# Zialus/CUDA-Recommender

Hardware: AMD Instinct MI355X
Metric: rating-nnz/sec per CCD++ outer iter at k=64 (higher is better)
Workload: dtype f32

## Files before the change

### cuda-recommender_amd/csrc/ccd_kernels.hip

```cpp
#include "ccd_kernels.hpp"

#include <algorithm>
#include <cstdlib>
#include <mutex>
#include <type_traits>

#include "flat_layout.hpp"

namespace mfx {
namespace {

constexpr int kBlock = 256;
constexpr uint32_t kPerSegLdsCap = 1024;

using u32x4 = __attribute__((ext_vector_type(4))) uint32_t;
using f32x4 = __attribute__((ext_vector_type(4))) float;
using u16x4 = __attribute__((ext_vector_type(4))) uint16_t;

template <int CTRL, int ROW_MASK = 0xF>
__device__ __forceinline__ float dpp_mov(float src) {
    return __builtin_bit_cast(float, __builtin_amdgcn_update_dpp(0, __builtin_bit_cast(int, src), CTRL, ROW_MASK, 0xF, true));
}
constexpr int kDppRowShr = 0x110, kDppWaveShr1 = 0x138, kDppBcast15 = 0x142, kDppBcast31 = 0x143;

__device__ __forceinline__ float wave_sum(float x) {
    const uint32_t lane = threadIdx.x & 63;
    x += dpp_mov<kDppRowShr + 1>(x);
    x += dpp_mov<kDppRowShr + 2>(x);
    x += dpp_mov<kDppRowShr + 4>(x);
    x += dpp_mov<kDppRowShr + 8>(x);
    const float r15 = dpp_mov<kDppBcast15, 0xA>(x);
    if (lane & 16) x += r15;
    const float r31 = dpp_mov<kDppBcast31, 0xC>(x);
    if (lane & 32) x += r31;
    return __builtin_bit_cast(float, __builtin_amdgcn_readlane(__builtin_bit_cast(int, x), 63));
}

__device__ __forceinline__ void seg_scan2(float& xg, float& xh, uint32_t lane, uint32_t dist) {
    const uint32_t in_row = lane & 15;
#define MFX_SCAN_STEP(D)                                                            \
    {                                                                               \
        const float yg = dpp_mov<kDppRowShr + D>(xg), yh = dpp_mov<kDppRowShr + D>(xh); \
        if (in_row >= D && dist >= D) { xg += yg; xh += yh; }                     \
    }
    MFX_SCAN_STEP(1) MFX_SCAN_STEP(2) MFX_SCAN_STEP(4) MFX_SCAN_STEP(8)
#undef MFX_SCAN_STEP
    {
        const float yg = dpp_mov<kDppBcast15, 0xA>(xg), yh = dpp_mov<kDppBcast15, 0xA>(xh);
        if ((lane & 16) && dist > in_row) { xg += yg; xh += yh; }
    }
    {
        const float yg = dpp_mov<kDppBcast31, 0xC>(xg), yh = dpp_mov<kDppBcast31, 0xC>(xh);
        if ((lane & 32) && dist > lane - 32) { xg += yg; xh += yh; }
    }
}

__device__ __forceinline__ float mul_rn(float a, float b) {
#pragma clang fp contract(off)
    return a * b;
}
__device__ __forceinline__ float add_rn(float a, float b) {
#pragma clang fp contract(off)
    return a + b;
}
__device__ __forceinline__ float sub_rn(float a, float b) {
#pragma clang fp contract(off)
    return a - b;
}

__global__ __launch_bounds__(kBlock) void k_sweep_wave(uint32_t nseg, const uint32_t* __restrict__ ptr,
                                                       const uint32_t* __restrict__ idx,
                                                       const float* __restrict__ val,
                                                       const float* __restrict__ vec,
                                                       float* __restrict__ g_out, float* __restrict__ h_out) {
    const uint32_t lane = threadIdx.x & 63;
    const uint32_t wave = (blockIdx.x * kBlock + threadIdx.x) >> 6;
    const uint32_t nwaves = (gridDim.x * kBlock) >> 6;
    for (uint32_t c = wave; c < nseg; c += nwaves) {
        const uint32_t lo = ptr[c], hi = ptr[c + 1];
        float g = 0.f, h = 0.f;
        for (uint32_t p = lo + lane; p < hi; p += 64) {
            const float x = vec[idx[p]];
            g += x * val[p];
            h += x * x;
        }
        g = wave_sum(g);
        h = wave_sum(h);
        if (lane == 0) {
            g_out[c] = g;
            h_out[c] = h;
        }
    }
}

__global__ __launch_bounds__(kBlock) void k_resid_wave(uint32_t nseg, const uint32_t* __restrict__ ptr,
                                                       const uint32_t* __restrict__ idx,
                                                       float* __restrict__ val,
                                                       const float* __restrict__ gathered,
                                                       const float* __restrict__ per_seg, int add) {
    const uint32_t lane = threadIdx.x & 63;
    const uint32_t wave = (blockIdx.x * kBlock + threadIdx.x) >> 6;
    const uint32_t nwaves = (gridDim.x * kBlock) >> 6;
    for (uint32_t c = wave; c < nseg; c += nwaves) {
        const uint32_t lo = ptr[c], hi = ptr[c + 1];
        const float b = per_seg[c];
        for (uint32_t p = lo + lane; p < hi; p += 64) {
            const float prod = mul_rn(gathered[idx[p]], b);
            val[p] = add ? add_rn(val[p], prod) : sub_rn(val[p], prod);
        }
    }
}

struct FlatArgs {
    const void* idx;
    float* val;
    const uint32_t* flags32;
    const uint32_t* hpre;
    const uint32_t* seg_of_rank;
    const uint32_t* wg_panel;
    uint32_t nspans;
    uint32_t tiles_per_span;
    uint32_t panel_rows;
    uint32_t gather_len;
    uint32_t nne;
    uint64_t nnz;
    const void* gather;
    const void* perseg;
    float2* part;
    float2* carry;
    int add;
    const uint32_t* wg_order;
    const uint32_t* wg_g0;
    const uint32_t* wg_g1;
    const uint32_t* expected;
    uint32_t* arrived;
    const uint32_t* orphans;
    uint32_t norphans, ngroups, panel_lanes;
    uint32_t nseg, npanels;
    const uint32_t* ptr_v;
    const uint32_t* rank_code;
    const uint32_t* seg_cnt;
    float lambda;
    float* out_vec;
    float2* pack2;
    const float* next_vec;
    float4* pack4;
    const float* gather_aux;
};

struct F3 { float x, y, z; };
template <typename S, typename G> __device__ __forceinline__ S to_slice(const G& g) { return g; }
template <> __device__ __forceinline__ F3 to_slice<F3, float4>(const float4& g) { return F3{g.x, g.y, g.z}; }
template <typename G, typename S> __device__ __forceinline__ G from_slice(const S& s) { return s; }
template <> __device__ __forceinline__ float4 from_slice<float4, F3>(const F3& s) { return make_float4(s.x, s.y, s.z, 0.f); }
template <int MODE> struct ModeTraits;
template <> struct ModeTraits<FM_SWEEP> { using G = float;  using S = float;  using P = float;  static constexpr bool kPerSeg = false, kWrite = false, kDot = true, kAux = false; };
template <> struct ModeTraits<FM_RESID> { using G = float;  using S = float;  using P = float;  static constexpr bool kPerSeg = true,  kWrite = true,  kDot = false, kAux = false; };
template <> struct ModeTraits<FM_FCSC>  { using G = float2; using S = float2; using P = float2; static constexpr bool kPerSeg = true,  kWrite = true,  kDot = true, kAux = false; };
template <> struct ModeTraits<FM_FCSR>  { using G = float4; using S = F3;     using P = float2; static constexpr bool kPerSeg = true,  kWrite = true,  kDot = true, kAux = false; };
template <> struct ModeTraits<FM_FCSC_RO> { using G = float2; using S = float2; using P = float2; static constexpr bool kPerSeg = true, kWrite = false, kDot = true, kAux = false; };
template <> struct ModeTraits<FM_FCSR_RO> { using G = float4; using S = F3;     using P = float2; static constexpr bool kPerSeg = true, kWrite = false, kDot = true, kAux = false; };
template <> struct ModeTraits<FM_FCSC2> { using G = float4; using S = float4; using P = float4; static constexpr bool kPerSeg = true,  kWrite = true,  kDot = true, kAux = false; };
template <> struct ModeTraits<FM_FCSR2> { using G = float4; using S = float4; using P = float4; static constexpr bool kPerSeg = true,  kWrite = true,  kDot = true, kAux = true; };

__device__ __forceinline__ float zero_of(float) { return 0.f; }
__device__ __forceinline__ float2 zero_of(float2) { return make_float2(0.f, 0.f); }
__device__ __forceinline__ float4 zero_of(float4) { return make_float4(0.f, 0.f, 0.f, 0.f); }

template <int MODE>
__device__ __forceinline__ void element_op(float v, const typename ModeTraits<MODE>::G& ga, float aux,
                                           const typename ModeTraits<MODE>::P& ps, int add,
                                           float& v_out, float& gc, float& hc) {
    if constexpr (MODE == FM_SWEEP) {
        v_out = v;
        gc = ga * v;
        hc = ga * ga;
    } else if constexpr (MODE == FM_RESID) {
        const float prod = mul_rn(ga, ps);
        v_out = add ? add_rn(v, prod) : sub_rn(v, prod);
        gc = 0.f;
        hc = 0.f;
    } else if constexpr (MODE == FM_FCSC || MODE == FM_FCSC_RO) {
        v_out = add_rn(sub_rn(v, mul_rn(ga.x, ps.x)), mul_rn(ga.y, ps.y));
        gc = ga.y * v_out;
        hc = ga.y * ga.y;
    } else if constexpr (MODE == FM_FCSR || MODE == FM_FCSR_RO) {
        v_out = add_rn(sub_rn(v, mul_rn(ga.x, ps.x)), mul_rn(ga.y, ps.y));
        gc = ga.z * v_out;
        hc = ga.z * ga.z;
    } else {
        const float r = add_rn(sub_rn(v, mul_rn(ga.x, ps.x)), mul_rn(ga.y, ps.y));
        v_out = add_rn(sub_rn(r, mul_rn(ga.z, ps.z)), mul_rn(ga.w, ps.w));
        const float d = MODE == FM_FCSC2 ? ga.w : aux;
        gc = d * v_out;
        hc = d * d;
    }
}

template <int BLOCK> __device__ void fused_finalize(const FlatArgs& a, uint32_t chunk, unsigned char* lds_raw);

using gu64 = __attribute__((address_space(1))) unsigned long long;
using gu32 = __attribute__((address_space(1))) uint32_t;
template <bool FUSE>
__device__ __forceinline__ void store_partial(float2* p, float g, float h) {
    if constexpr (FUSE) {
        const unsigned long long bits = (unsigned long long) __builtin_bit_cast(uint32_t, g) | ((unsigned long long) __builtin_bit_cast(uint32_t, h) << 32);
        __hip_atomic_store((gu64*) p, bits, __ATOMIC_RELAXED, __HIP_MEMORY_SCOPE_AGENT);
    } else {
        *p = make_float2(g, h);
    }
}
__device__ __forceinline__ float2 load_partial_sc1(const float2* p) {
    const unsigned long long bits = __hip_atomic_load((gu64*) p, __ATOMIC_RELAXED, __HIP_MEMORY_SCOPE_AGENT);
    return make_float2(__builtin_bit_cast(float, (uint32_t) bits), __builtin_bit_cast(float, (uint32_t) (bits >> 32)));
}

template <int MODE> constexpr int flat_min_waves(int block) { return MODE == FM_FCSC_RO || MODE == FM_FCSR_RO ? block / 128 : 1; }

#ifndef MFX_RO_PERSIST_FORM
#define MFX_RO_PERSIST_FORM 1
#endif
template <int MODE, bool LDS, int BLOCK, bool PSCHK, bool FUSE = false, bool PERSIST = false>
__global__ __launch_bounds__(BLOCK, flat_min_waves<MODE>(BLOCK)) void k_flat(FlatArgs a) {
    static_assert(!FUSE || ModeTraits<MODE>::kDot, "fused finalize: passes that produce sums");
    static_assert(!PERSIST || (LDS && !FUSE), "persistent form: LDS panels without the in-pass finalize");
    using TR = ModeTraits<MODE>;
    constexpr bool ROP = PERSIST && !TR::kWrite;
    constexpr bool PERSIST2 = PERSIST && TR::kWrite;
    uint32_t chunk = FUSE ? a.wg_order[blockIdx.x] : blockIdx.x;
    uint32_t chunk_end = chunk + 1;
    const uint32_t nchunks = a.nspans / (BLOCK / 64);
    if constexpr (PERSIST) {
        chunk = (uint32_t) ((uint64_t) blockIdx.x * nchunks / gridDim.x);
        chunk_end = (uint32_t) ((uint64_t) (blockIdx.x + 1) * nchunks / gridDim.x);
        if (chunk >= chunk_end) return;
    }
    using G = typename TR::G;
    using P = typename TR::P;
    extern __shared__ __attribute__((aligned(16))) unsigned char lds_raw[];
    using S = typename TR::S;
    S* __restrict__ slice = reinterpret_cast<S*>(lds_raw);
    constexpr size_t kSliceEntry = sizeof(S) + (TR::kAux ? sizeof(float) : 0);
    float* __restrict__ aux_slice = reinterpret_cast<float*>(lds_raw + ((size_t) a.panel_rows + 1) * sizeof(S));
    const uint32_t lane = threadIdx.x & 63;
    uint32_t span = __builtin_amdgcn_readfirstlane(chunk * (BLOCK / 64) + (threadIdx.x >> 6));
    const G* __restrict__ gather = static_cast<const G*>(a.gather);
    const P* __restrict__ perseg = static_cast<const P*>(a.perseg);
    const uint32_t span_words = a.tiles_per_span * (kTileElems / 32);
    uint64_t start = (uint64_t) span * a.tiles_per_span * kTileElems;
    using IdxVec = typename std::conditional<LDS, u16x4, u32x4>::type;
    using IdxElem = typename std::conditional<LDS, uint16_t, uint32_t>::type;
    const IdxVec* __restrict__ idx4 = reinterpret_cast<const IdxVec*>(static_cast<const IdxElem*>(a.idx) + start) + lane;
    f32x4* __restrict__ val4 = reinterpret_cast<f32x4*>(a.val + start) + lane;
    const uint32_t* __restrict__ flw = a.flags32 + (size_t) span * span_words + (lane >> 3);
    const uint32_t* __restrict__ hpw = a.hpre + (size_t) span * span_words + (lane >> 3);
    const uint32_t sh = (lane & 7) * 4;
    IdxVec id_n;
    f32x4 v_n;
    uint32_t fl_n, hp_n, hp_nn;
    const size_t span_step_q = (size_t) (BLOCK / 64) * a.tiles_per_span * 64, span_step_w = (size_t) (BLOCK / 64) * span_words;
    uint64_t sq = ROP ? (uint64_t) span * a.tiles_per_span * 64 : 0, sw = ROP ? (uint64_t) span * span_words : 0;
    struct LaneOff { uint32_t i, v, w; };
    auto lane_off = [](uint32_t lane) { LaneOff o{lane * (uint32_t) sizeof(IdxVec), lane * 16u, (lane >> 3) * 4u}; asm volatile("" : "+v"(o.i), "+v"(o.v), "+v"(o.w)); return o; };
    using gchar = __attribute__((address_space(1))) const char;
    auto ubase = [](const void* p) {
        const uint64_t u = reinterpret_cast<uint64_t>(p);
        return reinterpret_cast<gchar*>((uint64_t) (uint32_t) __builtin_amdgcn_readfirstlane((int) (u >> 32)) << 32 | (uint32_t) __builtin_amdgcn_readfirstlane((int) u));
    };
    using GIdxVec = __attribute__((address_space(1))) const IdxVec;
    using GF32x4 = __attribute__((address_space(1))) const f32x4;
    auto ld_idx = [&](uint64_t q, uint32_t lane_ib) { return __builtin_nontemporal_load(reinterpret_cast<GIdxVec*>(ubase(static_cast<const IdxVec*>(a.idx) + (sq + q)) + lane_ib)); };
    auto ld_val = [&](uint64_t q, uint32_t lane_vb) { return __builtin_nontemporal_load(reinterpret_cast<GF32x4*>(ubase(reinterpret_cast<const f32x4*>(a.val) + (sq + q)) + lane_vb)); };
    auto ld_fl = [&](uint64_t w, uint32_t lane_wb) { return *reinterpret_cast<const gu32*>(ubase(a.flags32 + (sw + w)) + lane_wb); };
    auto ld_hp = [&](uint64_t w, uint32_t lane_wb) { return *reinterpret_cast<const gu32*>(ubase(a.hpre + (sw + w)) + lane_wb); };
    auto stage_slice = [&](uint32_t panel) {
        const uint32_t gbase = panel * a.panel_rows;
        const uint32_t cnt = a.gather_len - gbase < a.panel_rows ? a.gather_len - gbase : a.panel_rows;
        for (uint32_t i = threadIdx.x; i < cnt; i += BLOCK) slice[i] = to_slice<S, G>(gather[gbase + i]);
        if (threadIdx.x == 0) slice[a.panel_rows] = S{};
        if constexpr (TR::kAux) {
            for (uint32_t i = threadIdx.x; i < cnt; i += BLOCK) aux_slice[i] = a.gather_aux[gbase + i];
            if (threadIdx.x == 0) aux_slice[a.panel_rows] = 0.f;
        }
    };
    uint32_t panel = 0, panel_next = 0;
    if constexpr (LDS) {
        id_n = __builtin_nontemporal_load(idx4);
        v_n = __builtin_nontemporal_load(val4);
        fl_n = flw[0]; hp_n = hpw[0]; hp_nn = hpw[8];
        panel = a.wg_panel[chunk];
        stage_slice(panel);
    }
    P* __restrict__ ps_lds = reinterpret_cast<P*>(lds_raw + (((size_t) a.panel_rows + 1) * kSliceEntry + 15) / 16 * 16);
    uint32_t win_base = 0;
    auto heads_before = [&](uint32_t c) { return a.hpre[(size_t) c * (BLOCK / 64) * span_words]; };
    uint32_t hb1 = 0, hb2 = 0;
    if constexpr (LDS && TR::kPerSeg) {
        const uint32_t rb0 = heads_before(chunk);
        win_base = rb0 > 0 ? rb0 - 1 : 0;
        const uint32_t win_end = heads_before(chunk + 1);
        if constexpr (PERSIST2) { hb1 = win_end; hb2 = heads_before(chunk + 2 < nchunks ? chunk + 2 : nchunks); }
        uint32_t cnt = win_end - win_base;
        if (cnt > kPerSegLdsCap) cnt = kPerSegLdsCap;
        for (uint32_t j = threadIdx.x; j < cnt; j += BLOCK) ps_lds[j] = perseg[a.seg_of_rank[win_base + j]];
    }
    if constexpr (LDS && !PERSIST) __syncthreads();
    for (uint32_t visit = 0;; ++visit) {
    const bool more = PERSIST && chunk + 1 < chunk_end;
    uint32_t win_base_n = 0, win_cnt_n = 0;
    if constexpr (ROP) __syncthreads();
    if constexpr (PERSIST2) {
        if (visit && panel_next != panel) {
            __syncthreads();
            panel = panel_next;
            stage_slice(panel);
        }
        __syncthreads();
        if constexpr (TR::kPerSeg) {
            if (more) {
                win_base_n = hb1 > 0 ? hb1 - 1 : 0;
                win_cnt_n = hb2 - win_base_n < kPerSegLdsCap ? hb2 - win_base_n : kPerSegLdsCap;
            }
        }
    }
    P* __restrict__ ps_cur = PERSIST2 ? ps_lds + (visit & 1u) * kPerSegLdsCap : ps_lds;
    bool live = span < a.nspans;
    if constexpr (!FUSE) { if (!live) return; }
    auto fetch_ps = [&](uint32_t r) -> P {
        if constexpr (LDS) {
            const uint32_t rl = r - win_base;
            if constexpr (!PSCHK) return ps_cur[rl];
            else if (rl < kPerSegLdsCap) return ps_cur[rl];
        }
        return perseg[a.seg_of_rank[r]];
    };
    uint32_t ntiles = a.tiles_per_span;
    if constexpr (!LDS) {
        const uint64_t left = a.nnz > start ? a.nnz - start : 0;
        const uint32_t nlive = (uint32_t) ((left + kTileElems - 1) / kTileElems);
        if (nlive < ntiles) ntiles = nlive;
        if (live && ntiles == 0) {
            if (TR::kDot && lane == 0) store_partial<FUSE>(a.carry + span, 0.f, 0.f);
            live = false;
        }
        if constexpr (!FUSE) { if (!live) return; }
        if (live) {
            id_n = __builtin_nontemporal_load(idx4);
            v_n = __builtin_nontemporal_load(val4);
            fl_n = flw[0]; hp_n = hpw[0]; hp_nn = hpw[8];
        }
    }
    if (live) {
    const uint32_t rank_base = __builtin_amdgcn_readfirstlane(hp_n);
    uint32_t cur1 = rank_base;
    P pcur{};
    if constexpr (TR::kPerSeg) {
        if (cur1 > 0) pcur = fetch_ps(cur1 - 1);
    }
    float og = 0.f, oh = 0.f;
    bool open_spread = false;

    for (uint32_t tile = 0; tile < ntiles; ++tile) {
        const IdxVec id = id_n;
        const f32x4 v = v_n;
        const uint32_t fl = fl_n, hp = hp_n;
        const uint32_t cur1_next = __builtin_amdgcn_readfirstlane(hp_nn);
        hp_n = hp_nn;
        if constexpr (ROP) {
            const bool hop = MFX_RO_PERSIST_FORM == 2 && more && tile + 1 == ntiles;
            const uint64_t q = hop ? (uint64_t) span_step_q : (uint64_t) (tile + 1) * 64;
            const uint64_t w = hop ? (uint64_t) span_step_w : (uint64_t) (tile + 1) * 8;
            const LaneOff lo = lane_off(lane);
            if (hop || tile + 1 < ntiles) {
                id_n = ld_idx(q, lo.i);
                v_n = ld_val(q, lo.v);
            }
            fl_n = ld_fl(w, lo.w);
            hp_nn = ld_hp(w + 8, lo.w);
        } else if constexpr (!PERSIST) {
            if (tile + 1 < ntiles) {
                id_n = __builtin_nontemporal_load(idx4 + (tile + 1) * 64);
                v_n = __builtin_nontemporal_load(val4 + (tile + 1) * 64);
            }
            fl_n = flw[(tile + 1) * 8];
            hp_nn = hpw[(tile + 2) * 8];
        } else if (tile + 1 < ntiles) {
            id_n = __builtin_nontemporal_load(idx4 + (tile + 1) * 64);
            v_n = __builtin_nontemporal_load(val4 + (tile + 1) * 64);
            fl_n = flw[(tile + 1) * 8];
            hp_nn = hpw[(tile + 2) * 8];
        } else if (more) {
            id_n = __builtin_nontemporal_load(idx4 + span_step_q);
            v_n = __builtin_nontemporal_load(val4 + span_step_q);
            fl_n = flw[span_step_w]; hp_n = hpw[span_step_w]; hp_nn = hpw[span_step_w + 8];
            panel_next = a.wg_panel[chunk + 1];
            if constexpr (TR::kPerSeg) { hb1 = hb2; hb2 = heads_before(chunk + 3 < nchunks ? chunk + 3 : nchunks); }
        }
        const uint64_t base = start + (uint64_t) tile * kTileElems;
        const bool partial = !LDS && base + kTileElems > a.nnz;
        const uint64_t e0 = base + (uint64_t) lane * 4;

        const uint32_t ids[4] = {(uint32_t) id.x, (uint32_t) id.y, (uint32_t) id.z, (uint32_t) id.w};
        const float vs[4] = {v.x, v.y, v.z, v.w};
        G ga[4];
        float gx[4] = {};
#pragma unroll
        for (int e = 0; e < 4; ++e) {
            if constexpr (LDS) ga[e] = from_slice<G, S>(slice[ids[e]]);
            else ga[e] = ids[e] < a.gather_len ? gather[ids[e]] : zero_of(G{});
            if constexpr (LDS && TR::kAux) gx[e] = aux_slice[ids[e]];
        }
        float vo[4], gc[4], hc[4];

        if (cur1_next == cur1) {
#pragma unroll
            for (int e = 0; e < 4; ++e) {
                element_op<MODE>(vs[e], ga[e], gx[e], pcur, a.add, vo[e], gc[e], hc[e]);
                if (partial && e0 + e >= a.nnz) { gc[e] = 0.f; hc[e] = 0.f; }
                if constexpr (TR::kDot) { og += gc[e]; oh += hc[e]; }
            }
            open_spread = true;
        } else {
            const uint32_t nib = (fl >> sh) & 0xFu;
            const uint32_t r1 = hp + (uint32_t) __popc(fl & ((1u << sh) - 1u));
#pragma unroll
            for (int e = 0; e < 4; ++e) {
                P ps{};
                if constexpr (TR::kPerSeg) {
                    const uint32_t re1 = r1 + (uint32_t) __popc(nib & ((2u << e) - 1u));
                    ps = fetch_ps(re1 - 1);
                }
                element_op<MODE>(vs[e], ga[e], gx[e], ps, a.add, vo[e], gc[e], hc[e]);
                if (partial && e0 + e >= a.nnz) { gc[e] = 0.f; hc[e] = 0.f; }
            }
            if constexpr (TR::kDot) {
                float cin_g, cin_h;
                if (open_spread) {
                    cin_g = wave_sum(og);
                    cin_h = wave_sum(oh);
                } else {
                    cin_g = __builtin_bit_cast(float, __builtin_amdgcn_readfirstlane(__builtin_bit_cast(int, og)));
                    cin_h = __builtin_bit_cast(float, __builtin_amdgcn_readfirstlane(__builtin_bit_cast(int, oh)));
                }
                open_spread = false;
                float ag = 0.f, ah = 0.f, fg = 0.f, fh = 0.f;
                bool seen = false;
                uint32_t close1 = r1;
#pragma unroll
                for (int e = 0; e < 4; ++e) {
                    if ((nib >> e) & 1u) {
                        if (!seen) {
                            fg = ag; fh = ah; seen = true;
                        } else {
                            store_partial<FUSE>(a.part + (close1 - 1), ag, ah);
                        }
                        ++close1;
                        ag = 0.f; ah = 0.f;
                    }
                    ag += gc[e];
                    ah += hc[e];
                }
                if (!seen) { fg = ag; fh = ah; }
                const uint64_t M = __ballot(seen);
                const uint64_t upto = M & ((uint64_t(2) << lane) - 1);
                const uint32_t dist = upto ? lane - (63u - (uint32_t) __clzll((long long) upto)) : 64u;
                float xg = ag, xh = ah;
                seg_scan2(xg, xh, lane, dist);
                float eg = dpp_mov<kDppWaveShr1>(xg), eh = dpp_mov<kDppWaveShr1>(xh);
                if ((M & ((uint64_t(1) << lane) - 1)) == 0) { eg += cin_g; eh += cin_h; }
                if (seen) {
                    const float tg = eg + fg, th = eh + fh;
                    if (r1 > rank_base) {
                        store_partial<FUSE>(a.part + (r1 - 1), tg, th);
                    } else {
                        store_partial<FUSE>(a.carry + span, tg, th);
                    }
                }
                const float ng = __builtin_bit_cast(float, __builtin_amdgcn_readlane(__builtin_bit_cast(int, xg), 63));
                const float nh = __builtin_bit_cast(float, __builtin_amdgcn_readlane(__builtin_bit_cast(int, xh), 63));
                og = lane == 0 ? ng : 0.f;
                oh = lane == 0 ? nh : 0.f;
            }
            cur1 = cur1_next;
            if constexpr (TR::kPerSeg) pcur = fetch_ps(cur1 - 1);
        }
        if constexpr (TR::kWrite) {
            if (!partial) {
__builtin_nontemporal_store(f32x4{vo[0], vo[1], vo[2], vo[3]}, val4 + tile * 64);
            } else {
                float* vp = a.val + e0;
#pragma unroll
                for (int e = 0; e < 4; ++e)
                    if (e0 + e < a.nnz) vp[e] = vo[e];
            }
        }
    }
    if constexpr (TR::kDot) {
        const float tg = open_spread ? wave_sum(og) : og, th = open_spread ? wave_sum(oh) : oh;
        if (lane == 0) {
            if (cur1 > rank_base) {
                store_partial<FUSE>(a.part + (cur1 - 1), tg, th);
            } else {
                store_partial<FUSE>(a.carry + span, tg, th);
            }
        }
    }
    }
    if constexpr (!PERSIST) break;
    if (!more) break;
    if constexpr (ROP) {
        ++chunk;
        span += BLOCK / 64;
        sq += span_step_q;
        sw += span_step_w;
        const LaneOff lo = lane_off(lane);
        if (MFX_RO_PERSIST_FORM != 2) {
            id_n = ld_idx(0, lo.i);
            v_n = ld_val(0, lo.v);
            fl_n = ld_fl(0, lo.w); hp_nn = ld_hp(8, lo.w);
        }
        hp_n = ld_hp(0, lo.w);
        panel_next = a.wg_panel[chunk];
        const uint32_t rb0 = heads_before(chunk), win_end = heads_before(chunk + 1);
        __syncthreads();
        if (panel_next != panel) {
            panel = panel_next;
            stage_slice(panel);
        }
        win_base = rb0 > 0 ? rb0 - 1 : 0;
        const uint32_t cnt = win_end - win_base < kPerSegLdsCap ? win_end - win_base : kPerSegLdsCap;
        for (uint32_t j = threadIdx.x; j < cnt; j += BLOCK) ps_lds[j] = perseg[a.seg_of_rank[win_base + j]];
        continue;
    }
    if constexpr (TR::kPerSeg) {
        P* __restrict__ ps_nxt = ps_lds + ((visit + 1) & 1u) * kPerSegLdsCap;
        for (uint32_t j = threadIdx.x; j < win_cnt_n; j += BLOCK) ps_nxt[j] = perseg[a.seg_of_rank[win_base_n + j]];
        win_base = win_base_n;
    }
    ++chunk;
    span += BLOCK / 64;
    start = (uint64_t) span * a.tiles_per_span * kTileElems;
    idx4 = reinterpret_cast<const IdxVec*>(static_cast<const IdxElem*>(a.idx) + start) + lane;
    val4 = reinterpret_cast<f32x4*>(a.val + start) + lane;
    flw = a.flags32 + (size_t) span * span_words + (lane >> 3);
    hpw = a.hpre + (size_t) span * span_words + (lane >> 3);
    }
    if constexpr (FUSE) fused_finalize<BLOCK>(a, chunk, lds_raw);
}


constexpr uint32_t kSegOwnerLong = 1024;
#ifndef MFX_OWNER_UL
#define MFX_OWNER_UL 2
#define MFX_OWNER_US 1
#endif
#ifndef MFX_SEG_BLOCK
#define MFX_SEG_BLOCK 256
#endif
constexpr int kSegBlock = MFX_SEG_BLOCK;
struct SegOwnerArgs {
    const uint32_t* ptr;
    const uint32_t* idx;
    float* val;
    const void* gather;
    const void* perseg;
    const uint4* long_list;
    const uint4* short_list;
    uint32_t nlong, nshort;
    float lambda;
    float* out_vec;
    float2* pack2;
    const float* next_vec;
    float4* pack4;
};

template <int MODE>
__device__ __forceinline__ void seg_owner_finish(const SegOwnerArgs& a, uint32_t c, uint32_t cnt, float g, float h,
                                                 const typename ModeTraits<MODE>::P& ps, float next_old) {
    const float x = cnt ? g / add_rn(mul_rn(a.lambda, (float) cnt), h) : 0.f;
    a.out_vec[c] = x;
    if constexpr (MODE == FM_FCSC || MODE == FM_FCSR) {
        if (a.pack4) a.pack4[c] = make_float4(ps.x, ps.y, x, 0.f);
        a.pack2[c] = make_float2(x, a.next_vec == a.out_vec ? x : next_old);
    }
}

template <int MODE>
__global__ __launch_bounds__(kSegBlock) void k_seg_owner(SegOwnerArgs a) {
    using TR = ModeTraits<MODE>;
    using G = typename TR::G;
    using P = typename TR::P;
    const G* __restrict__ gather = static_cast<const G*>(a.gather);
    const P* __restrict__ perseg = static_cast<const P*>(a.perseg);
    const uint32_t lane = threadIdx.x & 63, wave = threadIdx.x >> 6;
    __shared__ float sg[kSegBlock / 64], sh[kSegBlock / 64];
    auto walk = [&](uint32_t lo, uint32_t hi, uint32_t first, uint32_t stride, const P& ps, float& g, float& h, auto unroll) {
        constexpr int U = decltype(unroll)::value;
        g = 0.f; h = 0.f;
        if (hi == lo) return;
        const uint32_t base = lo & ~3u;
        uint32_t pq[U];
        u32x4 id4[U];
        f32x4 v4[U];
        auto streams = [&](uint32_t p0, uint32_t (&pp)[U], u32x4 (&ii)[U], f32x4 (&vals)[U]) {
#pragma unroll
            for (int u = 0; u < U; ++u) {
                pp[u] = p0 + (uint32_t) u * 4u * stride;
                const uint32_t at = pp[u] < hi ? pp[u] : base;
                ii[u] = *reinterpret_cast<const u32x4*>(a.idx + at);
                vals[u] = *reinterpret_cast<const f32x4*>(a.val + at);
            }
        };
        uint32_t p = base + 4u * first;
        if (p < hi) streams(p, pq, id4, v4);
        while (p < hi) {
            G ga[U][4];
#pragma unroll
            for (int u = 0; u < U; ++u)
#pragma unroll
                for (int e = 0; e < 4; ++e) ga[u][e] = gather[id4[u][e]];
            const uint32_t pn = p + 4u * stride * U;
            uint32_t pqn[U];
            u32x4 id4n[U];
            f32x4 v4n[U];
            if (pn < hi) streams(pn, pqn, id4n, v4n);
#pragma unroll
            for (int u = 0; u < U; ++u) {
                f32x4 o;
                bool all_live = true;
#pragma unroll
                for (int e = 0; e < 4; ++e) {
                    const uint32_t pos = pq[u] + (uint32_t) e;
                    const bool live = pos >= lo && pos < hi;
                    all_live &= live;
                    float vo, gc, hc;
                    element_op<MODE>(v4[u][e], ga[u][e], 0.f, ps, 0, vo, gc, hc);
                    o[e] = vo;
                    g += live ? gc : 0.f; h += live ? hc : 0.f;
                }
                if constexpr (TR::kWrite) {
                    if (all_live) {
                        *reinterpret_cast<f32x4*>(a.val + pq[u]) = o;
                    } else if (pq[u] < hi) {
#pragma unroll
                        for (int e = 0; e < 4; ++e) { const uint32_t pos = pq[u] + (uint32_t) e; if (pos >= lo && pos < hi) a.val[pos] = o[e]; }
                    }
                }
            }
            p = pn;
            if (p < hi) {
#pragma unroll
                for (int u = 0; u < U; ++u) { pq[u] = pqn[u]; id4[u] = id4n[u]; v4[u] = v4n[u]; }
            }
        }
    };
    if (blockIdx.x < a.nlong) {
        const uint4 e = a.long_list[blockIdx.x];
        const uint32_t c = e.x, lo = e.y, hi = e.z;
        P ps{};
        if constexpr (TR::kPerSeg) ps = perseg[c];
        float g, h;
        walk(lo, hi, threadIdx.x, kSegBlock, ps, g, h, std::integral_constant<int, MFX_OWNER_UL>{});
        g = wave_sum(g); h = wave_sum(h);
        if (lane == 0) { sg[wave] = g; sh[wave] = h; }
        __syncthreads();
        if (threadIdx.x == 0) {
            float tg = 0.f, th = 0.f;
            for (int w = 0; w < kSegBlock / 64; ++w) { tg += sg[w]; th += sh[w]; }
            seg_owner_finish<MODE>(a, c, hi - lo, tg, th, ps, a.next_vec ? a.next_vec[c] : 0.f);
        }
        return;
    }
    const uint32_t nwaves = (gridDim.x - a.nlong) * (kSegBlock / 64);
    for (uint32_t q = (blockIdx.x - a.nlong) * (kSegBlock / 64) + wave; q < a.nshort; q += nwaves) {
        const uint4 e = a.short_list[q];
        const uint32_t c = e.x, lo = e.y, hi = e.z;
        P ps{};
        if constexpr (TR::kPerSeg) ps = perseg[c];
        const float next_old = a.next_vec ? a.next_vec[c] : 0.f;
        float g, h;
        walk(lo, hi, lane, 64, ps, g, h, std::integral_constant<int, MFX_OWNER_US>{});
        g = wave_sum(g); h = wave_sum(h);
        if (lane == 0) seg_owner_finish<MODE>(a, c, hi - lo, g, h, ps, next_old);
    }
}

template <bool SC1>
__device__ __forceinline__ float2 load_partial(const float2* p) {
    if constexpr (SC1) return load_partial_sc1(p);
    else return *p;
}
template <bool SC1 = false>
__device__ __forceinline__ void add_carries(uint32_t lo, uint32_t hi, uint32_t span_len, const float2* __restrict__ carry,
                                            float& g, float& h) {
    uint32_t s = lo / span_len + 1;
    const uint32_t s_end = (hi - 1) / span_len;
    for (; s + 3 <= s_end; s += 4) {
        const float2 c0 = load_partial<SC1>(carry + s), c1 = load_partial<SC1>(carry + s + 1), c2 = load_partial<SC1>(carry + s + 2),
                     c3 = load_partial<SC1>(carry + s + 3);
        g += c0.x; g += c1.x; g += c2.x; g += c3.x;
        h += c0.y; h += c1.y; h += c2.y; h += c3.y;
    }
    for (; s <= s_end; ++s) { const float2 c = load_partial<SC1>(carry + s); g += c.x; h += c.y; }
}

struct GatherPartsArgs {
    uint32_t nseg, npanels, span_len;
    const uint32_t* ptr_v;
    const uint32_t* rank_code;
    const float2* part;
    const float2* carry;
};
constexpr uint32_t kNoRank = 0xFFFFFFFFu, kCarryBit = 0x80000000u;

template <bool SC1 = false>
__device__ __forceinline__ void segment_sums(const GatherPartsArgs& a, uint32_t c, uint32_t p0, uint32_t stride,
                                             float& g, float& h) {
    constexpr int kBatch = 5;
    g = 0.f;
    h = 0.f;
    for (uint32_t pb = p0; pb < a.npanels; pb += stride * kBatch) {
        uint32_t r[kBatch];
#pragma unroll
        for (int q = 0; q < kBatch; ++q) {
            const uint32_t p = pb + q * stride;
            r[q] = p < a.npanels ? a.rank_code[(size_t) p * a.nseg + c] : kNoRank;
        }
        float2 pp[kBatch];
#pragma unroll
        for (int q = 0; q < kBatch; ++q) pp[q] = r[q] != kNoRank ? load_partial<SC1>(a.part + (r[q] & ~kCarryBit)) : make_float2(0.f, 0.f);
#pragma unroll
        for (int q = 0; q < kBatch; ++q) {
            if (r[q] != kNoRank) {
                if (r[q] & kCarryBit) {
                    const size_t v = (size_t) (pb + q * stride) * a.nseg + c;
                    add_carries<SC1>(a.ptr_v[v], a.ptr_v[v + 1], a.span_len, a.carry, pp[q].x, pp[q].y);
                }
                g += pp[q].x;
                h += pp[q].y;
            }
        }
    }
}

template <int PL>
__device__ __forceinline__ bool block_segment_sums(const GatherPartsArgs& a, uint32_t& c, float& g, float& h) {
    constexpr int SEGS = kBlock / PL;
    __shared__ float sg[kBlock], sh[kBlock];
    const uint32_t sl = threadIdx.x % SEGS, pl = threadIdx.x / SEGS;
    c = blockIdx.x * SEGS + sl;
    g = 0.f;
    h = 0.f;
    if (c < a.nseg) segment_sums(a, c, pl, PL, g, h);
    if constexpr (PL > 1) {
        sg[threadIdx.x] = g;
        sh[threadIdx.x] = h;
        __syncthreads();
        if (pl == 0) {
            for (int q = 1; q < PL; ++q) { g += sg[q * SEGS + sl]; h += sh[q * SEGS + sl]; }
        }
    }
    return pl == 0 && c < a.nseg;
}

template <int PL>
__global__ __launch_bounds__(kBlock) void k_combine_dense(GatherPartsArgs a, float* __restrict__ gh) {
    uint32_t c;
    float g, h;
    if (!block_segment_sums<PL>(a, c, g, h)) return;
    gh[c] = g;
    gh[a.nseg + c] = h;
}

struct FinKernelArgs {
    GatherPartsArgs parts;
    const uint32_t* seg_cnt;
    const float* gh_dense;
    uint32_t seg_base, gh_len;
    const unsigned long long* slab_acc;
    const uint32_t* slab_lo;
    const uint32_t* slab_bad;
    uint32_t slab_pr;
    const uint32_t* cnt_override;
    float lambda;
    float* out_vec;
    float2* pack2;
    const float* next_vec;
    float4* pack4;
    bool pack4_as3;
    bool nmf;
    double* fundec_seg;
    float4* quad;
};

template <int PL>
__global__ __launch_bounds__(kBlock) void k_finalize(FinKernelArgs a) {
    constexpr int SEGS = kBlock / PL;
    const bool flat = !a.gh_dense && !a.slab_acc;
    const uint32_t dl = blockIdx.x * kBlock + threadIdx.x;
    const uint32_t c0 = flat ? blockIdx.x * SEGS + threadIdx.x % SEGS : a.seg_base + dl;
    const bool owner = flat ? (c0 < a.parts.nseg && threadIdx.x / SEGS == 0) : dl < a.gh_len;
    uint32_t cnt = 0;
    float2 old = make_float2(0.f, 0.f);
    float next = 0.f;
    if (owner) {
        cnt = a.cnt_override ? a.cnt_override[c0] : a.seg_cnt[c0];
        if (a.pack2) { old = a.pack2[c0]; next = a.next_vec[c0]; }
    }
    uint32_t c;
    float g, h;
    if (a.slab_acc) {
        c = c0;
        if (dl >= a.gh_len) return;
        const uint32_t p = c / a.slab_pr, l = c - p * a.slab_pr;
        unsigned long long ig = 0, ih = 0;
        uint32_t bad = 0;
        for (uint32_t w = a.slab_lo[p]; w < a.slab_lo[p + 1]; ++w) {
            const unsigned long long* sl = a.slab_acc + (size_t) w * 2 * a.slab_pr + 2 * l;
            ig += sl[0]; ih += sl[1];
            bad |= a.slab_bad[w];
        }
        constexpr double inv = 1.0 / 68719476736.0;
        g = bad ? __builtin_nanf("") : (float) ((double) (long long) ig * inv);
        h = bad ? __builtin_nanf("") : (float) ((double) (long long) ih * inv);
    } else if (a.gh_dense) {
        c = c0;
        if (dl >= a.gh_len) return;
        g = a.gh_dense[dl];
        h = a.gh_dense[a.gh_len + dl];
    } else if (!block_segment_sums<PL>(a.parts, c, g, h)) {
        return;
    }
    const float den = add_rn(mul_rn(a.lambda, (float) cnt), h);
    float x = cnt ? g / den : 0.f;
    if (a.nmf || a.fundec_seg) {
        const float was = a.pack2 ? old.y : a.out_vec[c];
        double fd = 0.0;
        if (cnt) {
            if (a.nmf && x < 0.f) {
                x = 0.f;
// ... 580 lines not shown
```

Before: 4.544 billion.

## Batch and overlap LDS panel staging with per-segment window gathers

Replaces the simple strided loops that stage gather slices and per-segment windows into LDS with batched register loads. Up to eight loads per thread are issued before the LDS writes, and the window gathers are interleaved with panel staging. In the persistent write path, the next panel is staged ahead before the barrier so the global latency overlaps prior work. Launch bounds for FM_FCSR now ask for more waves per EU. This raises register pressure and adds clamped redundant loads, and the reordered syncs carry some risk of LDS races.

New measurement: 4.558 billion (median of 2 runs). Within noise of the previous version (+0.3%).

```diff
diff --git a/cuda-recommender_amd/csrc/ccd_kernels.hip b/cuda-recommender_amd/csrc/ccd_kernels.hip
--- a/cuda-recommender_amd/csrc/ccd_kernels.hip
+++ b/cuda-recommender_amd/csrc/ccd_kernels.hip
@@ -15,6 +15,8 @@
 
 using u32x4 = __attribute__((ext_vector_type(4))) uint32_t;
 using f32x4 = __attribute__((ext_vector_type(4))) float;
+using f32x2 = __attribute__((ext_vector_type(2))) float;
+using f32x3 = __attribute__((ext_vector_type(3))) float;
 using u16x4 = __attribute__((ext_vector_type(4))) uint16_t;
 
 template <int CTRL, int ROW_MASK = 0xF>
@@ -149,8 +151,6 @@
 };
 
 struct F3 { float x, y, z; };
-template <typename S, typename G> __device__ __forceinline__ S to_slice(const G& g) { return g; }
-template <> __device__ __forceinline__ F3 to_slice<F3, float4>(const float4& g) { return F3{g.x, g.y, g.z}; }
 template <typename G, typename S> __device__ __forceinline__ G from_slice(const S& s) { return s; }
 template <> __device__ __forceinline__ float4 from_slice<float4, F3>(const F3& s) { return make_float4(s.x, s.y, s.z, 0.f); }
 template <int MODE> struct ModeTraits;
@@ -215,11 +215,21 @@
     return make_float2(__builtin_bit_cast(float, (uint32_t) bits), __builtin_bit_cast(float, (uint32_t) (bits >> 32)));
 }
 
-template <int MODE> constexpr int flat_min_waves(int block) { return MODE == FM_FCSC_RO || MODE == FM_FCSR_RO ? block / 128 : 1; }
+template <int MODE> constexpr int flat_min_waves(int block) { return MODE == FM_FCSC_RO || MODE == FM_FCSR_RO || MODE == FM_FCSR ? block / 128 : 1; }
 
 #ifndef MFX_RO_PERSIST_FORM
 #define MFX_RO_PERSIST_FORM 1
 #endif
+#ifndef MFX_STAGE_AHEAD
+#define MFX_STAGE_AHEAD 1
+#endif
+#ifndef MFX_RO_STAGE_AHEAD
+#define MFX_RO_STAGE_AHEAD 0
+#endif
+#ifndef MFX_RO_WINDOW_FIRST
+#define MFX_RO_WINDOW_FIRST 0
+#endif
+constexpr int kStageBatch = 8;
 template <int MODE, bool LDS, int BLOCK, bool PSCHK, bool FUSE = false, bool PERSIST = false>
 __global__ __launch_bounds__(BLOCK, flat_min_waves<MODE>(BLOCK)) void k_flat(FlatArgs a) {
     static_assert(!FUSE || ModeTraits<MODE>::kDot, "fused finalize: passes that produce sums");
@@ -273,14 +283,64 @@
     auto ld_val = [&](uint64_t q, uint32_t lane_vb) { return __builtin_nontemporal_load(reinterpret_cast<GF32x4*>(ubase(reinterpret_cast<const f32x4*>(a.val) + (sq + q)) + lane_vb)); };
     auto ld_fl = [&](uint64_t w, uint32_t lane_wb) { return *reinterpret_cast<const gu32*>(ubase(a.flags32 + (sw + w)) + lane_wb); };
     auto ld_hp = [&](uint64_t w, uint32_t lane_wb) { return *reinterpret_cast<const gu32*>(ubase(a.hpre + (sw + w)) + lane_wb); };
-    auto stage_slice = [&](uint32_t panel) {
-        const uint32_t gbase = panel * a.panel_rows;
-        const uint32_t cnt = a.gather_len - gbase < a.panel_rows ? a.gather_len - gbase : a.panel_rows;
-        for (uint32_t i = threadIdx.x; i < cnt; i += BLOCK) slice[i] = to_slice<S, G>(gather[gbase + i]);
-        if (threadIdx.x == 0) slice[a.panel_rows] = S{};
-        if constexpr (TR::kAux) {
-            for (uint32_t i = threadIdx.x; i < cnt; i += BLOCK) aux_slice[i] = a.gather_aux[gbase + i];
-            if (threadIdx.x == 0) aux_slice[a.panel_rows] = 0.f;
+    using GN = typename std::conditional<sizeof(S) == 16, f32x4, typename std::conditional<sizeof(S) == 12, f32x3,
+               typename std::conditional<sizeof(S) == 8, f32x2, float>::type>::type>::type;
+    struct StageBatch { GN g[kStageBatch]; float x[TR::kAux ? kStageBatch : 1]; };
+    auto slice_cnt = [&](uint32_t panel) { const uint32_t gbase = panel * a.panel_rows; return a.gather_len - gbase < a.panel_rows ? a.gather_len - gbase : a.panel_rows; };
+    auto stage_tid = []() { uint32_t t = threadIdx.x; asm volatile("" : "+v"(t)); return t; };
+    auto stage_issue = [&](uint32_t panel, uint32_t cnt, uint32_t first, StageBatch& r) {
+        gchar* gb = ubase(gather + panel * a.panel_rows);
+        gchar* xb = nullptr;
+        if constexpr (TR::kAux) xb = ubase(a.gather_aux + panel * a.panel_rows);
+        const uint32_t t = stage_tid();
+#pragma unroll
+        for (int b = 0; b < kStageBatch; ++b) {
+            const uint32_t i = first + t + (uint32_t) b * BLOCK, ic = i < cnt ? i : cnt - 1;
+            r.g[b] = *reinterpret_cast<const __attribute__((address_space(1))) GN*>(gb + ic * (uint32_t) sizeof(G));
+            if constexpr (TR::kAux) r.x[b] = *reinterpret_cast<const __attribute__((address_space(1))) float*>(xb + ic * 4u);
+        }
+    };
+    auto stage_commit = [&](uint32_t cnt, uint32_t first, const StageBatch& r) {
+        const uint32_t t = stage_tid();
+#pragma unroll
+        for (int b = 0; b < kStageBatch; ++b) {
+            const uint32_t i = first + t + (uint32_t) b * BLOCK;
+            if (i < cnt) {
+                if constexpr (sizeof(S) == 12) slice[i] = S{r.g[b].x, r.g[b].y, r.g[b].z};
+                else slice[i] = __builtin_bit_cast(S, r.g[b]);
+                if constexpr (TR::kAux) aux_slice[i] = r.x[b];
+            }
+        }
+        if (first == 0 && threadIdx.x == 0) {
+            slice[a.panel_rows] = S{};
+            if constexpr (TR::kAux) aux_slice[a.panel_rows] = 0.f;
+        }
+    };
+    auto stage_rest = [&](uint32_t panel, uint32_t cnt) {
+        for (uint32_t first = kStageBatch * BLOCK; first < cnt; first += kStageBatch * BLOCK) {
+            StageBatch r;
+            stage_issue(panel, cnt, first, r);
+            stage_commit(cnt, first, r);
+        }
+    };
+    constexpr int kWinBatch = (kPerSegLdsCap + BLOCK - 1) / BLOCK;
+    using PN = typename std::conditional<sizeof(P) == 16, f32x4, typename std::conditional<sizeof(P) == 8, f32x2, float>::type>::type;
+    auto win_issue = [&](uint32_t wb, uint32_t cnt, uint32_t (&sg)[kWinBatch]) {
+#pragma unroll
+        for (int b = 0; b < kWinBatch; ++b) {
+            const uint32_t j = threadIdx.x + (uint32_t) b * BLOCK;
+            sg[b] = a.seg_of_rank[wb + (j < cnt ? j : cnt ? cnt - 1 : 0)];
+        }
+    };
+    auto win_gather = [&](const uint32_t (&sg)[kWinBatch], PN (&pv)[kWinBatch]) {
+#pragma unroll
+        for (int b = 0; b < kWinBatch; ++b) pv[b] = reinterpret_cast<const PN*>(perseg)[sg[b]];
+    };
+    auto win_commit = [&](P* __restrict__ dst, uint32_t cnt, const PN (&pv)[kWinBatch]) {
+#pragma unroll
+        for (int b = 0; b < kWinBatch; ++b) {
+            const uint32_t j = threadIdx.x + (uint32_t) b * BLOCK;
+            if (j < cnt) reinterpret_cast<PN*>(dst)[j] = pv[b];
         }
     };
     uint32_t panel = 0, panel_next = 0;
@@ -288,21 +348,31 @@
         id_n = __builtin_nontemporal_load(idx4);
         v_n = __builtin_nontemporal_load(val4);
         fl_n = flw[0]; hp_n = hpw[0]; hp_nn = hpw[8];
-        panel = a.wg_panel[chunk];
-        stage_slice(panel);
     }
     P* __restrict__ ps_lds = reinterpret_cast<P*>(lds_raw + (((size_t) a.panel_rows + 1) * kSliceEntry + 15) / 16 * 16);
     uint32_t win_base = 0;
     auto heads_before = [&](uint32_t c) { return a.hpre[(size_t) c * (BLOCK / 64) * span_words]; };
     uint32_t hb1 = 0, hb2 = 0;
-    if constexpr (LDS && TR::kPerSeg) {
-        const uint32_t rb0 = heads_before(chunk);
-        win_base = rb0 > 0 ? rb0 - 1 : 0;
-        const uint32_t win_end = heads_before(chunk + 1);
-        if constexpr (PERSIST2) { hb1 = win_end; hb2 = heads_before(chunk + 2 < nchunks ? chunk + 2 : nchunks); }
-        uint32_t cnt = win_end - win_base;
-        if (cnt > kPerSegLdsCap) cnt = kPerSegLdsCap;
-        for (uint32_t j = threadIdx.x; j < cnt; j += BLOCK) ps_lds[j] = perseg[a.seg_of_rank[win_base + j]];
+    if constexpr (LDS) {
+        panel = a.wg_panel[chunk];
+        uint32_t wcnt = 0;
+        if constexpr (TR::kPerSeg) {
+            const uint32_t rb0 = heads_before(chunk);
+            const uint32_t win_end = heads_before(chunk + 1);
+            if constexpr (PERSIST2) { hb1 = win_end; hb2 = heads_before(chunk + 2 < nchunks ? chunk + 2 : nchunks); }
+            win_base = __builtin_amdgcn_readfirstlane(rb0 > 0 ? rb0 - 1 : 0);
+            wcnt = win_end - win_base < kPerSegLdsCap ? win_end - win_base : kPerSegLdsCap;
+        }
+        uint32_t sg[kWinBatch];
+        PN pv[kWinBatch];
+        if constexpr (TR::kPerSeg) win_issue(win_base, wcnt, sg);
+        const uint32_t cnt = slice_cnt(panel);
+        StageBatch sb;
+        stage_issue(panel, cnt, 0, sb);
+        if constexpr (TR::kPerSeg) win_gather(sg, pv);
+        stage_commit(cnt, 0, sb);
+        stage_rest(panel, cnt);
+        if constexpr (TR::kPerSeg) win_commit(ps_lds, wcnt, pv);
     }
     if constexpr (LDS && !PERSIST) __syncthreads();
     for (uint32_t visit = 0;; ++visit) {
@@ -310,10 +380,14 @@
     uint32_t win_base_n = 0, win_cnt_n = 0;
     if constexpr (ROP) __syncthreads();
     if constexpr (PERSIST2) {
-        if (visit && panel_next != panel) {
+        if (!MFX_STAGE_AHEAD && visit && panel_next != panel) {
             __syncthreads();
             panel = panel_next;
-            stage_slice(panel);
+            const uint32_t cnt = slice_cnt(panel);
+            StageBatch sb;
+            stage_issue(panel, cnt, 0, sb);
+            stage_commit(cnt, 0, sb);
+            stage_rest(panel, cnt);
         }
         __syncthreads();
         if constexpr (TR::kPerSeg) {
@@ -513,29 +587,67 @@
         span += BLOCK / 64;
         sq += span_step_q;
         sw += span_step_w;
-        const LaneOff lo = lane_off(lane);
-        if (MFX_RO_PERSIST_FORM != 2) {
-            id_n = ld_idx(0, lo.i);
-            v_n = ld_val(0, lo.v);
-            fl_n = ld_fl(0, lo.w); hp_nn = ld_hp(8, lo.w);
-        }
-        hp_n = ld_hp(0, lo.w);
+        auto first_tile = [&]() {
+            const LaneOff lo = lane_off(lane);
+            if (MFX_RO_PERSIST_FORM != 2) {
+                id_n = ld_idx(0, lo.i);
+                v_n = ld_val(0, lo.v);
+                fl_n = ld_fl(0, lo.w); hp_nn = ld_hp(8, lo.w);
+            }
+            hp_n = ld_hp(0, lo.w);
+        };
+        if (!MFX_RO_WINDOW_FIRST) first_tile();
         panel_next = a.wg_panel[chunk];
         const uint32_t rb0 = heads_before(chunk), win_end = heads_before(chunk + 1);
-        __syncthreads();
-        if (panel_next != panel) {
+        win_base = rb0 > 0 ? rb0 - 1 : 0;
+        const uint32_t wcnt = win_end - win_base < kPerSegLdsCap ? win_end - win_base : kPerSegLdsCap;
+        const bool restage = panel_next != panel;
+        constexpr bool kAhead = MFX_RO_STAGE_AHEAD || MFX_RO_WINDOW_FIRST;
+        uint32_t sg[kWinBatch];
+        PN pv[kWinBatch];
+        if (kAhead) win_issue(win_base, wcnt, sg);
+        if (MFX_RO_WINDOW_FIRST) {
+            win_gather(sg, pv);
+            first_tile();
+        }
+        if (restage) {
+            const uint32_t cnt = slice_cnt(panel_next);
+            StageBatch sb;
+            if (MFX_RO_STAGE_AHEAD) stage_issue(panel_next, cnt, 0, sb);
+            __syncthreads();
+            if (!kAhead) win_issue(win_base, wcnt, sg);
+            if (!MFX_RO_STAGE_AHEAD) stage_issue(panel_next, cnt, 0, sb);
+            if (!MFX_RO_WINDOW_FIRST) win_gather(sg, pv);
             panel = panel_next;
-            stage_slice(panel);
-        }
-        win_base = rb0 > 0 ? rb0 - 1 : 0;
-        const uint32_t cnt = win_end - win_base < kPerSegLdsCap ? win_end - win_base : kPerSegLdsCap;
-        for (uint32_t j = threadIdx.x; j < cnt; j += BLOCK) ps_lds[j] = perseg[a.seg_of_rank[win_base + j]];
+            stage_commit(cnt, 0, sb);
+            stage_rest(panel, cnt);
+        } else {
+            __syncthreads();
+            if (!kAhead) win_issue(win_base, wcnt, sg);
+            if (!MFX_RO_WINDOW_FIRST) win_gather(sg, pv);
+        }
+        win_commit(ps_lds, wcnt, pv);
         continue;
     }
-    if constexpr (TR::kPerSeg) {
+    {
+        const bool restage = MFX_STAGE_AHEAD && panel_next != panel;
+        uint32_t sg[kWinBatch];
+        PN pv[kWinBatch];
         P* __restrict__ ps_nxt = ps_lds + ((visit + 1) & 1u) * kPerSegLdsCap;
-        for (uint32_t j = threadIdx.x; j < win_cnt_n; j += BLOCK) ps_nxt[j] = perseg[a.seg_of_rank[win_base_n + j]];
-        win_base = win_base_n;
+        if constexpr (TR::kPerSeg) { win_issue(win_base_n, win_cnt_n, sg); win_base = win_base_n; }
+        if (restage) {
+            const uint32_t cnt = slice_cnt(panel_next);
+            StageBatch sb;
+            stage_issue(panel_next, cnt, 0, sb);
+            if constexpr (TR::kPerSeg) { win_gather(sg, pv); win_commit(ps_nxt, win_cnt_n, pv); }
+            __syncthreads();
+            panel = panel_next;
+            stage_commit(cnt, 0, sb);
+            stage_rest(panel, cnt);
+        } else if constexpr (TR::kPerSeg) {
+            win_gather(sg, pv);
+            win_commit(ps_nxt, win_cnt_n, pv);
+        }
     }
     ++chunk;
     span += BLOCK / 64;
```
